# supranational/sppark

Hardware: AMD Instinct MI355X
Metric: MSM points/sec (BLS12-381 G1, 2^26 points) (higher is better)
Workload: dtype u32

## Files before the change

### sppark_amd/csrc/msm/msm_driver.hpp

```cpp
#pragma once
#include "msm_kernels.hpp"
#include "msm_coop_kernels.hpp"
#include "msm_route.hpp"
#include "../ec/jacobian_host.hpp"
#include "../util/runtime.hpp"
#include <algorithm>
#include <cmath>
#include <map>
#include <mutex>
#include <vector>

namespace sppark_amd {

template<class FD, class FH, class FRp>
class msm_t {
public:
    typedef FD fp_d;
    static constexpr bool G2_COOP_BUILT = field_is_internal<FD>::value && !field_is_montx<FD>::value;
    typedef mont_dev<FRp> fr_d;
    typedef FH fp_h;
    typedef typename xyzz_dev<fp_d>::mem_t bucket_t;
    typedef jacobian_host<fp_h> point_t;
    static constexpr int STD_WORDS = sizeof(FH) / 4;
    static constexpr size_t FP_BYTES = sizeof(FH);
    static constexpr bool INTERNAL = field_is_internal<FD>::value;
    static constexpr bool MONTX = field_is_montx<FD>::value;
    typedef xyzz_mem<STD_WORDS> std_bucket_t;
    static_assert(INTERNAL || sizeof(FH) == 4 * FD::N, "host and device coordinate fields must share the wire image");
    static constexpr size_t SCALAR_BYTES = sizeof(fr_d);
    static constexpr unsigned MAX_WINS = 128;
    static msm_field field()
    {
        bool pairs_default = false;
        if constexpr (G2_COOP_BUILT) pairs_default = fp_d::NL >= 14;
        return msm_field{INTERNAL, MONTX, G2_COOP_BUILT, pairs_default, (unsigned)fp_d::N, (unsigned)sizeof(bucket_t), (unsigned)FP_BYTES,
                         FRp::MOD, (unsigned)FRp::N};
    }
    static constexpr size_t FIXED_BASE_MIN = (size_t)1 << 23;

private:
    const gpu_info* gpu;
    hipStream_t stream;
    bool own_stream;
    hipStream_t aux = nullptr;
    unsigned gseq = 0;
    hipStream_t cpy = nullptr;
    hipEvent_t join_ev = nullptr;
    hipEvent_t ev_fork = nullptr, ev_sorted[2] = {nullptr, nullptr}, ev_accdone[2] = {nullptr, nullptr};
    hipEvent_t ev_copied[2] = {nullptr, nullptr}, ev_chunkdone[2] = {nullptr, nullptr};
    unsigned char* blob = nullptr;
    size_t blob_sz = 0;
    unsigned char* stage = nullptr;
    size_t stage_sz = 0;
    std_bucket_t* h_sums = nullptr;
    size_t h_sums_cap = 0;
    u32* h_flag = nullptr;
    const u32* h_flag_cur = nullptr;
    u32* d_pflag = nullptr;
    bool piece_pending = false;
    std::vector<hipEvent_t> tev;
    unsigned char* pre_points = nullptr;
    size_t pre_n = 0, pre_stride = 0;
    unsigned pre_fb_wbits = 0, pre_fb_nwins = 0;
    float last_ms[4] = {0, 0, 0, 0};
    unsigned last_chunks = 0;
    unsigned last_redo = 0;
    bool timing = false;

    struct layout {
        size_t digits[2], sorted[2], partA[2], H[2], tot[2], offA[2], off[2], curB[2], bigl[2];
        size_t buckets, keyA, ptA, keyB, ptB, keyC, flag, A1, W1, A2, W2, conv, sums, total;
    };

    static size_t align_up(size_t x) { return (x + 255) & ~(size_t)255; }
    static constexpr size_t conv_stride()
    {
        if constexpr (INTERNAL) return affine_loader<FD>::STRIDE; else return 0;
    }

    layout make_layout(const msm_plan& p, bool convert) const
    {
        layout l; size_t o = 0;
        auto take = [&](size_t sz) { size_t r = o; o += align_up(sz); return r; };
        const size_t wg = p.wpg;
        for (unsigned b = 0; b < 2; b++) {
            if (b == 1 && p.G == 1) {
                l.digits[1] = l.digits[0]; l.sorted[1] = l.sorted[0]; l.partA[1] = l.partA[0]; l.H[1] = l.H[0]; l.tot[1] = l.tot[0];
                l.offA[1] = l.offA[0]; l.off[1] = l.off[0]; l.curB[1] = l.curB[0]; l.bigl[1] = l.bigl[0];
                break;
            }
            l.digits[b] = take(wg * p.n * 4);
            l.sorted[b] = take(wg * p.n * 4);
            l.partA[b]  = take(wg * p.n * (p.IB ? 4 : 8));
            l.H[b]      = take(wg * p.nslabs * p.NA * 4);
            l.tot[b]    = take(wg * p.NA * 4);
            l.offA[b]   = take(wg * (p.NA + 1) * 4);
            l.off[b]    = take(wg * ((size_t)p.NB + 1) * 4);
            l.curB[b]   = take(wg * ((size_t)p.NB + 1) * 4);
            l.bigl[b]   = take((wg * p.NA + 1) * 4);
        }
        l.buckets = take((size_t)p.nwins * p.NB * sizeof(bucket_t));
        size_t nrecA = (size_t)2 * p.nwins * p.chunks_per_win;
        size_t nrecB = 2 * ((nrecA + p.F - 1) / p.F);
        l.keyA = take(nrecA * 4); l.ptA = take(nrecA * sizeof(bucket_t));
        l.keyB = take(nrecB * 4); l.ptB = take(nrecB * sizeof(bucket_t));
        l.keyC = take(nrecA * 4); l.flag = take(4);
        size_t n1 = (size_t)p.nwins * std::max<size_t>(p.NB / p.K1, lg2_floor(p.NB) + 1);
        l.A1 = take(n1 * sizeof(bucket_t)); l.W1 = take(n1 * sizeof(bucket_t));
        l.A2 = take(n1 * sizeof(bucket_t)); l.W2 = take(n1 * sizeof(bucket_t));
        l.conv = take(INTERNAL && convert ? (size_t)p.n * conv_stride() : 0);
        l.sums = take(((size_t)p.nwins + 1) * std::max(sizeof(std_bucket_t), sizeof(bucket_t)));
        l.total = o;
        return l;
    }

    void reserve(size_t sz)
    {
        if (sz <= blob_sz) return;
        if (blob) {
            HIP_OK(hipStreamSynchronize(stream));
            if (aux) HIP_OK(hipStreamSynchronize(aux));
            HIP_OK(hipFree(blob)); blob = nullptr; blob_sz = 0;
        }
        HIP_OK(dev_scratch_pool::malloc_or_drain((void**)&blob, sz));
        blob_sz = sz;
    }
    void reserve_stage(size_t sz)
    {
        if (sz <= stage_sz) return;
        if (stage) { HIP_OK(hipDeviceSynchronize()); HIP_OK(hipFree(stage)); stage = nullptr; stage_sz = 0; }
        HIP_OK(dev_scratch_pool::malloc_or_drain((void**)&stage, sz));
        stage_sz = sz;
    }
    void reserve_sums(size_t count)
    {
        if (count <= h_sums_cap) return;
        if (h_sums) { HIP_OK(hipStreamSynchronize(stream)); HIP_OK(hipHostFree(h_sums)); h_sums = nullptr; h_sums_cap = 0; }
        HIP_OK(hipHostMalloc((void**)&h_sums, count * sizeof(std_bucket_t), hipHostMallocDefault));
        h_sums_cap = count;
    }
    void need_event(hipEvent_t& e) { if (!e) HIP_OK(hipEventCreateWithFlags(&e, hipEventDisableTiming)); }
    std::map<const void*, size_t> lds_done;
    void lds_attr(const void* fn, size_t bytes)
    {
        size_t& have = lds_done[fn];
        if (bytes <= have) return;
        HIP_OK(hipFuncSetAttribute(fn, hipFuncAttributeMaxDynamicSharedMemorySize, (int)bytes));
        have = bytes;
    }
    void need_aux()
    {
        if (aux) return;
        unsigned ncu = 0;
#ifdef SPPARK_TUNING
        if (const char* e = getenv("SPPARK_MSM_AUX_CUS")) ncu = (unsigned)atoi(e);
#endif
        const unsigned total = (unsigned)gpu->prop.multiProcessorCount;
        hipError_t err = hipErrorNotSupported;
        if (ncu && ncu < total) {
            std::vector<uint32_t> mask((total + 31) / 32, 0);
            for (unsigned k = 0; k < ncu; k++) {
                unsigned cu = (unsigned)(((uint64_t)k * total) / ncu);
                mask[cu / 32] |= 1u << (cu % 32);
            }
            err = hipExtStreamCreateWithCUMask(&aux, (uint32_t)mask.size(), mask.data());
            if (err != hipSuccess) { (void)hipGetLastError(); aux = nullptr; }
        }
        if (!aux) HIP_OK(hipStreamCreateWithFlags(&aux, hipStreamNonBlocking));
        need_event(ev_fork);
        for (int b = 0; b < 2; b++) { need_event(ev_sorted[b]); need_event(ev_accdone[b]); }
    }
    void need_cpy()
    {
        if (cpy) return;
        HIP_OK(hipStreamCreateWithFlags(&cpy, hipStreamNonBlocking));
        for (int b = 0; b < 2; b++) { need_event(ev_copied[b]); need_event(ev_chunkdone[b]); }
    }
    void need_tev(size_t count)
    {
        while (tev.size() < count) { hipEvent_t e; HIP_OK(hipEventCreate(&e)); tev.push_back(e); }
    }

public:
    msm_tunables tune;

    explicit msm_t(int device_id = -1, hipStream_t s = nullptr)
        : gpu(&select_gpu(device_id)), stream(s), own_stream(false)
    {
        {
            int nb = 0, cur = -1;
            (void)hipGetDevice(&cur);
            if (cur != gpu->hip_id) HIP_OK(hipSetDevice(gpu->hip_id));
            if (hipOccupancyMaxActiveBlocksPerMultiprocessor(&nb, (const void*)k_accumulate<fp_d, false>, 256, 0) == hipSuccess && nb > 0)
                tune.resident_lanes = (size_t)std::min(nb, 2) * 256 * (size_t)gpu->prop.multiProcessorCount;
            else (void)hipGetLastError();
            if (cur >= 0 && cur != gpu->hip_id) (void)hipSetDevice(cur);
        }
        if constexpr (G2_COOP_BUILT) { if (fp_d::NL >= 14) tune.long_runs = 1; }
        if (stream == nullptr) {
            HIP_OK(hipStreamCreateWithFlags(&stream, hipStreamNonBlocking));
            HIP_OK(hipEventCreateWithFlags(&join_ev, hipEventDisableTiming));
            own_stream = true;
        }
    }
    ~msm_t()
    {
        int cur = -1;
        (void)hipGetDevice(&cur);
        if (cur != gpu->hip_id) (void)hipSetDevice(gpu->hip_id);
        (void)hipStreamSynchronize(stream);
        if (aux) (void)hipStreamSynchronize(aux);
        if (cpy) (void)hipStreamSynchronize(cpy);
        if (blob) (void)hipFree(blob);
        if (stage) (void)hipFree(stage);
        if (h_sums) (void)hipHostFree(h_sums);
        if (h_flag) (void)hipHostFree(h_flag);
        if (d_pflag) (void)hipFree(d_pflag);
        if (pre_points) (void)hipFree(pre_points);
        for (auto& e : tev) (void)hipEventDestroy(e);
        for (hipEvent_t e : {ev_fork, ev_sorted[0], ev_sorted[1], ev_accdone[0], ev_accdone[1],
                             ev_copied[0], ev_copied[1], ev_chunkdone[0], ev_chunkdone[1], join_ev})
            if (e) (void)hipEventDestroy(e);
        if (aux) (void)hipStreamDestroy(aux);
        if (cpy) (void)hipStreamDestroy(cpy);
        if (own_stream) (void)hipStreamDestroy(stream);
        if (cur >= 0 && cur != gpu->hip_id) (void)hipSetDevice(cur);
    }
    msm_t(const msm_t&) = delete;
    msm_t& operator=(const msm_t&) = delete;

    int device() const { return gpu->hip_id; }
    void set_stream(hipStream_t s)
    {
        (void)hipStreamSynchronize(stream);
        if (own_stream) { (void)hipStreamDestroy(stream); own_stream = false; }
        stream = s;
        if (stream == nullptr) {
            HIP_OK(hipStreamCreateWithFlags(&stream, hipStreamNonBlocking));
            if (!join_ev) HIP_OK(hipEventCreateWithFlags(&join_ev, hipEventDisableTiming));
            own_stream = true;
        }
    }
    void enable_timing(bool on) { timing = on; }
    float kernel_ms(int which) const { return which >= 0 && which < 4 ? last_ms[which] : -1.f; }
    unsigned chunks_of_last_invoke() const { return last_chunks; }
    unsigned tail_redone() const { return last_redo; }
    size_t scratch_bytes() const { return blob_sz + stage_sz; }
    void release_scratch()
    {
        (void)hipSetDevice(gpu->hip_id);
        (void)hipStreamSynchronize(stream);
        if (aux) (void)hipStreamSynchronize(aux);
        if (cpy) (void)hipStreamSynchronize(cpy);
        if (blob) { (void)hipFree(blob); blob = nullptr; blob_sz = 0; }
        if (stage) { (void)hipFree(stage); stage = nullptr; stage_sz = 0; }
    }
    msm_plan plan_for(size_t npoints) const { return make_plan(npoints, FRp::NBITS, tune); }

    void reserve_for(size_t npoints, size_t ffi_affine_sz, bool host_points, bool host_scalars)
    {
        HIP_OK(hipSetDevice(gpu->hip_id));
        size_t chunk = choose_chunk(npoints, (host_points ? ffi_affine_sz : 0) + (host_scalars ? SCALAR_BYTES : 0));
        const std::vector<size_t> cb = chunk_bounds(npoints, chunk);
        size_t need = 0;
        for (size_t c = 0; c + 1 < cb.size(); c++) need = std::max(need, make_layout(make_plan(cb[c + 1] - cb[c], FRp::NBITS, tune), true).total);
        reserve(need);
        if (host_points || host_scalars)
            reserve_stage(2 * (align_up(host_points ? chunk * ffi_affine_sz : 0) + align_up(host_scalars ? chunk * SCALAR_BYTES : 0)));
    }

    void join_default_stream()
    {
        if (!own_stream) return;
        HIP_OK(hipEventRecord(join_ev, nullptr));
        HIP_OK(hipStreamWaitEvent(stream, join_ev, 0));
    }

    unsigned fixed_base_width(size_t np) const
    {
        if (tune.wbits) return std::min(26u, std::max(8u, tune.wbits));
        unsigned w = 0; double best = 0;
        for (unsigned c = 8; c <= 26; c++) {
            const double cost = (double)((FRp::NBITS - 1) / c + 1) * (double)np + 3.0 * (double)((size_t)1 << (c - 1));
            if (w == 0 || cost < best) { best = cost; w = c; }
        }
        return w;
    }
    void preload(const void* points, size_t np, size_t ffi_affine_sz, bool fixed_base = false)
    {
        HIP_OK(hipSetDevice(gpu->hip_id));
        HIP_OK(hipStreamSynchronize(stream));
        join_default_stream();
        if (np != 0 && (points == nullptr || ffi_affine_sz < 2 * FP_BYTES || np > (1u << 31))) HIP_OK(hipErrorInvalidValue);
        if (np != 0 && fixed_base && !MONTX) HIP_OK(hipErrorNotSupported);
        if (np != 0 && fixed_base && (tune.wbits || np >= FIXED_BASE_MIN)
            && (size_t)((FRp::NBITS - 1) / fixed_base_width(np) + 1) * np >= ((size_t)1 << 31)) HIP_OK(hipErrorInvalidValue);
        if (pre_points) { HIP_OK(hipFree(pre_points)); pre_points = nullptr; pre_n = pre_stride = 0; }
        pre_fb_wbits = pre_fb_nwins = 0;
        if (np == 0) return;
        if (fixed_base && !MONTX) HIP_OK(hipErrorNotSupported);
        if (fixed_base && !tune.wbits && np < FIXED_BASE_MIN) fixed_base = false;
        unsigned fb_w = 0, fb_nw = 1;
        if (fixed_base) {
            fb_w = fixed_base_width(np);
            fb_nw = (FRp::NBITS - 1) / fb_w + 1;
            fb_w = FRp::NBITS / fb_nw + (FRp::NBITS % fb_nw ? 1 : 0);
            if ((size_t)fb_nw * np >= ((size_t)1 << 31)) HIP_OK(hipErrorInvalidValue);
        }
        if (points == nullptr || ffi_affine_sz < 2 * FP_BYTES || np > (1u << 31)) HIP_OK(hipErrorInvalidValue);
        struct dev_buf {
            unsigned char* p = nullptr;
            ~dev_buf() { if (p) (void)hipFree(p); }
        } staging;
        try {
            if constexpr (INTERNAL) {
                const unsigned char* src = (const unsigned char*)points;
                if (!is_device_pointer(points)) {
                    HIP_OK(hipMalloc((void**)&staging.p, np * ffi_affine_sz));
                    HIP_OK(hipMemcpyAsync(staging.p, points, np * ffi_affine_sz, hipMemcpyHostToDevice, stream));
                    src = staging.p;
                }
                HIP_OK(dev_scratch_pool::malloc_or_drain((void**)&pre_points, (size_t)fb_nw * np * conv_stride()));
                launch_convert(pre_points, src, (unsigned)np, ffi_affine_sz);
                if constexpr (MONTX) if (fixed_base) {
                    hipLaunchKernelGGL(k_fixed_base_table<fp_d>, dim3((unsigned)((np + 255) / 256)), dim3(256), 0, stream,
                                       pre_points, (unsigned)np, fb_nw, (unsigned)FRp::NBITS);
                    HIP_OK(hipGetLastError());
                }
            } else {
                HIP_OK(hipMalloc((void**)&pre_points, np * ffi_affine_sz));
                HIP_OK(hipMemcpyAsync(pre_points, points, np * ffi_affine_sz,
                                      is_device_pointer(points) ? hipMemcpyDeviceToDevice : hipMemcpyHostToDevice, stream));
            }
            HIP_OK(hipStreamSynchronize(stream));
        } catch (...) {
            if (pre_points) { (void)hipFree(pre_points); pre_points = nullptr; }
            throw;
        }
        pre_n = np; pre_stride = ffi_affine_sz;
        if (fixed_base) { pre_fb_wbits = fb_w; pre_fb_nwins = fb_nw; }
    }
    unsigned fixed_base_windows() const { return pre_fb_nwins; }
    size_t preloaded() const { return pre_n; }

private:
    static void no_kernel() { HIP_OK(hipErrorInvalidDeviceFunction); }
    void launch_convert(unsigned char* dst, const unsigned char* src, unsigned n, size_t stride, hipStream_t on = nullptr)
    {
        if constexpr (INTERNAL)
            issue_convert(route_convert(field(), tune.sw, n, stride, ((size_t)src & 15) == 0), dst, src, stride, on ? on : stream);
    }
    void issue_convert(const msm_step& s, unsigned char* dst, const unsigned char* src, size_t stride, hipStream_t on)
    {
        if constexpr (INTERNAL) {
            const dim3 grid(s.gx), block(s.block);
            switch (s.kernel) {
            case MK_CONVERT:         hipLaunchKernelGGL((k_convert_points<fp_d, false>), grid, block, 0, on, dst, src, s.count, (unsigned)stride); break;
            case MK_CONVERT_FLAGGED: hipLaunchKernelGGL((k_convert_points<fp_d, true>), grid, block, 0, on, dst, src, s.count, (unsigned)stride); break;
            case MK_CONVERT_STAGED:
                if constexpr (MONTX) hipLaunchKernelGGL((k_convert_points_staged<fp_d, false>), grid, block, 0, on, dst, src, s.count); else no_kernel();
                break;
            case MK_CONVERT_STAGED_FLAGGED:
                if constexpr (MONTX) hipLaunchKernelGGL((k_convert_points_staged<fp_d, true>), grid, block, 0, on, dst, src, s.count); else no_kernel();
                break;
            default: no_kernel();
            }
            HIP_OK(hipGetLastError());
        } else no_kernel();
    }

    size_t choose_chunk(size_t n, size_t stage_per_point) const
    {
        size_t chunk = n;
        if (tune.chunk) chunk = std::min(n, std::max<size_t>(tune.chunk, 1));
        else if (stage_per_point && n > ((size_t)1 << 21)) {
            chunk = std::min<size_t>(std::max<size_t>(n / 4, (size_t)1 << 20), (size_t)1 << 24);
        }
        auto need = [&](size_t c) {
            return make_layout(make_plan(c, FRp::NBITS, tune), true).total + 2 * c * stage_per_point + 1024;
        };
        size_t limit = tune.max_scratch;
        if (!limit) {
            const bool blob_ok = make_layout(make_plan(chunk, FRp::NBITS, tune), true).total <= blob_sz;
            const bool stage_ok = stage_per_point == 0 || 2 * (chunk * stage_per_point + 512) <= stage_sz;
            if (blob_ok && stage_ok) return chunk;
            size_t free_b = 0, total_b = 0;
            if (hipMemGetInfo(&free_b, &total_b) != hipSuccess) { (void)hipGetLastError(); return chunk; }
            limit = free_b - (free_b >> 5) + blob_sz + stage_sz;
        }
        while (need(chunk) > limit && chunk > 4096) chunk = (chunk + 1) / 2;
        return chunk;
    }

    std::vector<size_t> chunk_bounds(size_t n, size_t chunk) const
    {
        std::vector<size_t> b{0};
        for (size_t lo = chunk; lo < n; lo += chunk) b.push_back(lo);
        b.push_back(n);
        return b;
    }

    void sort_group(hipStream_t ss, const msm_plan& p, const layout& l, unsigned b, unsigned w0, unsigned wn,
                    const u32* d_scalars, bool mont, unsigned fb_n = 0, unsigned fb_nwins = 0)
    {
        u32* digits = (u32*)(blob + l.digits[b]);
        u32* sorted = (u32*)(blob + l.sorted[b]);
        u32* H = (u32*)(blob + l.H[b]);
        u32* tot = (u32*)(blob + l.tot[b]);
        u32* off = (u32*)(blob + l.off[b]);
        void* partA = blob + l.partA[b];
        u32* offA = (u32*)(blob + l.offA[b]);
        const bool packed = p.IB != 0;
        unsigned ngp = 1; while (ngp < p.NG) ngp <<= 1;
        const partA_fmt fmt{H, p.IB, p.SH, ngp, p.nslabs};
        const unsigned nlong = p.nbits % p.nwins, sf = nlong == 0 ? wn : (nlong > w0 ? std::min(wn, nlong - w0) : 0u);
        if (fb_n) {
            unsigned grid = std::min<unsigned>((fb_n + 255) / 256, 256 * 16);
            hipLaunchKernelGGL(k_breakdown<fr_d>, dim3(grid), dim3(256), 0, ss,
                               digits, d_scalars, fb_n, fb_nwins, (unsigned)FRp::NBITS, (int)mont, 0u, fb_nwins);
        } else {
            unsigned grid = std::min<unsigned>((p.n + 255) / 256, 256 * 16);
            hipLaunchKernelGGL(k_breakdown<fr_d>, dim3(grid), dim3(256), 0, ss,
                               digits, d_scalars, p.n, p.nwins, p.nbits, (int)mont, w0, wn);
        }
        HIP_OK(hipGetLastError());
        size_t ldsA = (size_t)p.NA * 4, ldsB = ((size_t)1 << p.LB) * 4 + SORT_NT * 4 + (size_t)SORTB_STAGE * 4 + PARTA_MAX_GROUPS * 4;
        if (ldsA > 65536) { lds_attr((const void*)k_histA, ldsA); lds_attr(packed ? (const void*)k_scatterA<true> : (const void*)k_scatterA<false>, ldsA); }
        if (ldsB > 65536) lds_attr(packed ? (const void*)k_sortB<true> : (const void*)k_sortB<false>, ldsB);
        hipLaunchKernelGGL(k_histA, dim3(p.nslabs, wn), dim3(SORT_NT), ldsA, ss,
                           H, digits, p.n, p.nslabs, p.slab_sz, p.NA, p.LB, sf);
        HIP_OK(hipGetLastError());
        size_t na_total = (size_t)wn * p.NA;
        hipLaunchKernelGGL(k_scan_slabs, dim3((unsigned)((na_total + 255) / 256)), dim3(256), 0, ss,
                           H, tot, p.nslabs, p.NA, wn);
        HIP_OK(hipGetLastError());
        hipLaunchKernelGGL(k_scan_parts, dim3(wn), dim3(1024), 0, ss, offA, tot, p.NA);
        HIP_OK(hipGetLastError());
        if (p.NA <= SCATA_MAX_NA && p.LB < 16) {
            const size_t ldsS = scatterA_staged_lds(p.NA);
            lds_attr(packed ? (const void*)k_scatterA_staged<true> : (const void*)k_scatterA_staged<false>, ldsS);
            if (packed) hipLaunchKernelGGL(k_scatterA_staged<true>, dim3(p.nslabs, wn), dim3(SORT_NT), ldsS, ss,
                                           (u32*)partA, digits, H, offA, p.n, p.nslabs, p.slab_sz, p.NA, p.LB, sf, p.IB);
            else        hipLaunchKernelGGL(k_scatterA_staged<false>, dim3(p.nslabs, wn), dim3(SORT_NT), ldsS, ss,
                                           (uint2*)partA, digits, H, offA, p.n, p.nslabs, p.slab_sz, p.NA, p.LB, sf, p.IB);
        } else {
            if (packed) hipLaunchKernelGGL(k_scatterA<true>, dim3(p.nslabs, wn), dim3(SORT_NT), ldsA, ss,
                                           (u32*)partA, digits, H, offA, p.n, p.nslabs, p.slab_sz, p.NA, p.LB, sf, p.IB);
            else        hipLaunchKernelGGL(k_scatterA<false>, dim3(p.nslabs, wn), dim3(SORT_NT), ldsA, ss,
                                           (uint2*)partA, digits, H, offA, p.n, p.nslabs, p.slab_sz, p.NA, p.LB, sf, p.IB);
        }
        HIP_OK(hipGetLastError());
        const unsigned big = tune.big ? tune.big : p.big ? p.big : (1u << 18);
        u32* nbig = (u32*)(blob + l.bigl[b]); u32* blist = nbig + 1; u32* curB = (u32*)(blob + l.curB[b]);
        const bool may_be_big = p.n > big;
        if (may_be_big) HIP_OK(hipMemsetAsync(nbig, 0, 4, ss));
        if (packed) hipLaunchKernelGGL(k_sortB<true>, dim3(p.NA, wn), dim3(SORT_NT), ldsB, ss,
                                       sorted, off, (const u32*)partA, offA, p.n, p.NA, p.LB, sf, big, fmt);
        else        hipLaunchKernelGGL(k_sortB<false>, dim3(p.NA, wn), dim3(SORT_NT), ldsB, ss,
                                       sorted, off, (const uint2*)partA, offA, p.n, p.NA, p.LB, sf, big, fmt);
        HIP_OK(hipGetLastError());
        if (!may_be_big) return;
        hipLaunchKernelGGL(k_big_find, dim3((p.NA * wn + 255) / 256), dim3(256), 0, ss,
                           nbig, blist, off, offA, p.NA, p.LB, sf, wn, big);
        size_t ldsBig = ((size_t)1 << p.LB) * 4;
        const size_t avg = (size_t)p.n / p.NA;
        const unsigned split = avg > big / 2 ? (unsigned)std::min<size_t>(SORTB_SPLIT, avg / (BIG_STAGE / 2) + 1) : SORTB_SPLIT;
        if (packed) hipLaunchKernelGGL(k_big_hist<true>, dim3(1024), dim3(1024), ldsBig, ss, off, (const u32*)partA, offA, nbig, blist, p.n, p.NA, p.LB, sf, split);
        else        hipLaunchKernelGGL(k_big_hist<false>, dim3(1024), dim3(1024), ldsBig, ss, off, (const uint2*)partA, offA, nbig, blist, p.n, p.NA, p.LB, sf, split);
        hipLaunchKernelGGL(k_big_scan, dim3(p.NA > 64 && avg > big / 2 ? 1024 : 64), dim3(1024), 0, ss, off, curB, offA, nbig, blist, p.NA, p.LB, sf);
        const size_t ldsSc = big_scatter_lds(p.LB);
        if (ldsSc > 65536) lds_attr(packed ? (const void*)k_big_scatter<true> : (const void*)k_big_scatter<false>, ldsSc);
        if (packed) hipLaunchKernelGGL(k_big_scatter<true>, dim3(1024), dim3(1024), ldsSc, ss, sorted, curB, (const u32*)partA, offA, nbig, blist, p.n, p.NA, p.LB, sf, split, fmt);
        else        hipLaunchKernelGGL(k_big_scatter<false>, dim3(1024), dim3(1024), ldsSc, ss, sorted, curB, (const uint2*)partA, offA, nbig, blist, p.n, p.NA, p.LB, sf, split, fmt);
        HIP_OK(hipGetLastError());
    }

    void enqueue(const msm_plan& p, const layout& l, const unsigned char* d_points, size_t stride, bool preconverted,
                 const u32* d_scalars, bool mont, std_bucket_t* h_out, bool first_timed, unsigned fb_n = 0, unsigned fb_nwins = 0,
                 bool redo = false, bool may_defer = false)
    {
        msm_call call;
        call.fb_n = fb_n; call.redo = redo; call.may_defer = may_defer;
        call.convert = INTERNAL && !preconverted;
        call.flagged = !preconverted && stride > 2 * FP_BYTES;
        call.stride = stride; call.aligned16 = ((size_t)d_points & 15) == 0;
#ifdef SPPARK_TUNING
        if (const char* e = getenv("SPPARK_TOP_CUT")) call.top_cut = (unsigned)atoi(e);
#endif
        const msm_route route = make_route(p, tune, field(), call);
        if (route.overflow) HIP_OK(hipErrorInvalidValue);
        const bool multi = p.G > 1;
        if (multi) need_aux();
        if (timing && first_timed && !redo) { need_tev(2 + 2 * p.G); HIP_OK(hipEventRecord(tev[0], stream)); }
        if (multi) {
            HIP_OK(hipEventRecord(ev_fork, stream));
            HIP_OK(hipStreamWaitEvent(aux, ev_fork, 0));
        }
        bucket_t* buckets = (bucket_t*)(blob + l.buckets);
        std_bucket_t* fin = (std_bucket_t*)(blob + l.sums);
        const u32* off0 = (const u32*)(blob + l.off[0]);
        auto rec = [&](msm_buf b) -> bucket_t* {
            switch (b) {
            case MB_BUCKETS: return buckets;
            case MB_PT_A: return (bucket_t*)(blob + l.ptA);
            case MB_PT_B: return (bucket_t*)(blob + l.ptB);
            case MB_A1: return (bucket_t*)(blob + l.A1);
            case MB_W1: return (bucket_t*)(blob + l.W1);
            case MB_A2: return (bucket_t*)(blob + l.A2);
            case MB_W2: return (bucket_t*)(blob + l.W2);
            default: return nullptr;
            }
        };
        auto key = [&](msm_buf b) -> u32* {
            return (u32*)(b == MB_KEY_A ? blob + l.keyA : b == MB_KEY_B ? blob + l.keyB : b == MB_KEY_C ? blob + l.keyC : nullptr);
        };
        auto flag_word = [&](msm_flag f) -> u32* { return f == MF_SCRATCH ? (u32*)(blob + l.flag) : f == MF_SMALL ? d_pflag : nullptr; };
        auto launch = [&](const msm_step& s, unsigned w0 = 0, unsigned wn = 0, unsigned b = 0) {
            const dim3 grid(s.gx, s.gy), block(s.block);
            bucket_t *r0 = rec(s.rd[0]), *r1 = rec(s.rd[1]), *w0p = rec(s.wr[0]), *w1p = rec(s.wr[1]);
            u32* flag = flag_word(s.flag);
            const u32* offp = multi ? (const u32*)nullptr : off0;
#define SPPARK_GO(kernel, ...) hipLaunchKernelGGL((kernel), grid, block, s.lds, stream, __VA_ARGS__)
#define SPPARK_GO_G1(kernel, ...) do { if constexpr (MONTX) SPPARK_GO(kernel, __VA_ARGS__); else no_kernel(); } while (0)
            switch (s.kernel) {
            case MK_CONVERT: case MK_CONVERT_FLAGGED: case MK_CONVERT_STAGED: case MK_CONVERT_STAGED_FLAGGED:
                issue_convert(s, blob + l.conv, d_points, stride, stream);
                return;
            case MK_ACCUMULATE: case MK_ACCUMULATE_FLAGGED: case MK_ACCUMULATE_G2C: {
                const u32* sorted = (const u32*)(blob + l.sorted[b]);
                const u32* off = (const u32*)(blob + l.off[b]);
                const dim3 rows(s.gx, wn);
                u32* keyA = key(MB_KEY_A); bucket_t* ptA = rec(MB_PT_A);
                if (s.kernel == MK_ACCUMULATE_G2C) {
                    if constexpr (G2_COOP_BUILT)
                        hipLaunchKernelGGL((k_accumulate_g2c<fp_d>), rows, block, 0, stream, buckets, keyA, ptA, d_points, (unsigned)stride,
                                           sorted, off, p.n, p.NB, p.L, p.chunks_per_win, w0);
                    else no_kernel();
                } else if (s.kernel == MK_ACCUMULATE_FLAGGED)
                    hipLaunchKernelGGL((k_accumulate<fp_d, true>), rows, block, 0, stream, buckets, keyA, ptA, d_points, (unsigned)stride,
                                       sorted, off, p.n, p.NB, p.L, p.chunks_per_win, w0);
                else
                    hipLaunchKernelGGL((k_accumulate<fp_d, false>), rows, block, 0, stream, buckets, keyA, ptA, d_points, (unsigned)stride,
                                       sorted, off, p.n, p.NB, p.L, p.chunks_per_win, w0);
                break;
            }
            case MK_PIECE_LEVEL:
                SPPARK_GO(k_piece_level<fp_d>, buckets, key(s.rd[0]), r1, off0, p.NB, p.L, p.chunks_per_win, p.nwins, route.piece_cmax, s.t, s.last, flag);
                break;
            case MK_PIECE_LEVEL_COOP:
                SPPARK_GO_G1(k_piece_level_coop<fp_d>, buckets, key(s.rd[0]), r1, off0, p.NB, p.L, p.chunks_per_win, p.nwins, route.piece_cmax, s.t, s.last, flag);
                break;
            case MK_PIECE_TAIL_COOP:
                SPPARK_GO_G1(k_piece_tail_coop<fp_d>, buckets, key(s.rd[0]), r1, off0, p.NB, p.L, p.chunks_per_win, p.nwins, route.piece_cmax, s.t, s.lgGB, flag);
                break;
            case MK_JOIN_RUNS:
                HIP_OK(hipMemsetAsync(flag, 0, 4, stream));
                SPPARK_GO(k_join_runs<fp_d>, buckets, key(s.wr[0]), key(s.rd[0]), r1, s.count, flag);
                break;
            case MK_REDUCE_RUNS:
                SPPARK_GO(k_reduce_runs<fp_d>, buckets, key(s.wr[0]), w1p, key(s.rd[0]), r1, s.count, s.fan, s.nthreads, (int)s.last, (const u32*)flag);
                break;
            case MK_REDUCE_RUNS_COOP:
                SPPARK_GO_G1(k_reduce_runs_coop<fp_d>, buckets, key(s.wr[0]), w1p, key(s.rd[0]), r1, s.count, s.fan, s.nthreads, 0, (const u32*)flag);
                break;
            case MK_REDUCE_TAIL:
                SPPARK_GO(k_reduce_tail<fp_d>, buckets, key(s.rd[0]), r1, key(s.wr[0]), w1p, s.count, s.fan, (const u32*)flag);
                break;
            case MK_REDUCE_TAIL_COOP:
                SPPARK_GO_G1(k_reduce_tail_coop<fp_d>, buckets, key(s.rd[0]), r1, key(s.wr[0]), w1p, s.count, s.fan, (const u32*)flag);
                break;
            case MK_BUCKET_SMALL_BITS_COOP: SPPARK_GO_G1(k_bucket_small_bits_coop<fp_d>, w0p, buckets, off0, p.NB, s.m); break;
            case MK_BUCKET_LEVEL1:      SPPARK_GO(k_bucket_level1<fp_d>, w0p, w1p, buckets, p.NB, s.fan, p.nwins, offp); break;
            case MK_BUCKET_LEVEL1_LAT:  SPPARK_GO_G1(k_bucket_level1_lat<fp_d>, w0p, w1p, buckets, p.NB, s.fan, p.nwins, offp); break;
            case MK_BUCKET_LEVEL1_PIPE: SPPARK_GO_G1(k_bucket_level1_pipe<fp_d>, w0p, w1p, buckets, p.NB, s.fan, p.nwins, offp); break;
            case MK_BUCKET_LEVEL1_COOP: SPPARK_GO_G1(k_bucket_level1_coop<fp_d>, w0p, w1p, buckets, p.NB, s.fan, p.nwins, offp); break;
            case MK_BUCKET_LEVELN:      SPPARK_GO(k_bucket_levelN<fp_d>, w0p, w1p, r0, r1, s.count, s.fan, s.lgG, p.nwins); break;
            case MK_BUCKET_LEVELN_LAT:  SPPARK_GO_G1(k_bucket_levelN_lat<fp_d>, w0p, w1p, r0, r1, s.count, s.fan, s.lgG, p.nwins); break;
            case MK_BUCKET_LEVELN_PIPE: SPPARK_GO_G1(k_bucket_levelN_pipe<fp_d>, w0p, w1p, r0, r1, s.count, s.fan, s.lgG, p.nwins); break;
            case MK_BUCKET_LEVELN_COOP: SPPARK_GO_G1(k_bucket_levelN_coop<fp_d>, w0p, w1p, r0, r1, s.count, s.fan, s.lgG, p.nwins); break;
            case MK_BUCKET_TOP_BITS:
                if (s.lds > 65536) lds_attr((const void*)k_bucket_top_bits<fp_d>, s.lds);
                SPPARK_GO(k_bucket_top_bits<fp_d>, w0p, r0, r1, s.count, s.m, s.lgG);
                break;
            case MK_BUCKET_TOP_SUM: SPPARK_GO(k_bucket_top_sum<fp_d>, w0p, r0, s.m); break;
            case MK_BUCKET_TOP_BITS_COOP:
                if constexpr (MONTX) { if (s.lds > 65536) lds_attr((const void*)k_bucket_top_bits_coop<fp_d>, s.lds); }
                SPPARK_GO_G1(k_bucket_top_bits_coop<fp_d>, w0p, r0, r1, s.count, s.m, s.lgG, s.sb, s.sp);
                break;
            case MK_BUCKET_TOP_SUM_COOP:
                SPPARK_GO_G1(k_bucket_top_sum_coop<fp_d>, w0p, r0, s.count, fin, flag, flag ? reinterpret_cast<u32*>(fin + p.nwins) : (u32*)nullptr);
                break;
            case MK_FINALIZE:
                if constexpr (INTERNAL) SPPARK_GO((k_finalize<fp_d, STD_WORDS>), fin, r0, p.nwins); else no_kernel();
                break;
            default: no_kernel();
            }
#undef SPPARK_GO_G1
#undef SPPARK_GO
            HIP_OK(hipGetLastError());
        };
        if (multi && !redo) HIP_OK(hipMemsetAsync(buckets, 0, (size_t)p.nwins * p.NB * sizeof(bucket_t), stream));

        for (unsigned g = 0; g < p.G && !redo; g++, gseq++) {
            const unsigned b = multi ? (gseq & 1) : 0, w0 = g * p.wpg, wn = std::min(p.wpg, p.nwins - w0);
            if (g == 0) {
                sort_group(stream, p, l, b, w0, wn, d_scalars, mont, fb_n, fb_nwins);
                if (call.convert) {
                    launch(route.steps[0]);
                    d_points = blob + l.conv;
                }
            } else {
                if (gseq >= 2) HIP_OK(hipStreamWaitEvent(aux, ev_accdone[b], 0));
                sort_group(aux, p, l, b, w0, wn, d_scalars, mont);
                HIP_OK(hipEventRecord(ev_sorted[b], aux));
                HIP_OK(hipStreamWaitEvent(stream, ev_sorted[b], 0));
            }
            if (timing && first_timed) HIP_OK(hipEventRecord(tev[2 + 2 * g], stream));
            launch(route.steps[route.front - 1], w0, wn, b);
            if (timing && first_timed) HIP_OK(hipEventRecord(tev[3 + 2 * g], stream));
            if (multi) HIP_OK(hipEventRecord(ev_accdone[b], stream));
        }

        unsigned si = route.front;
        piece_pending = route.piece_pending;
        if (route.flag_with_sums && !d_pflag) {
            HIP_OK(hipMalloc((void**)&d_pflag, 64));
            HIP_OK(hipMemsetAsync(d_pflag, 0, 64, stream));
        }
        if (route.pieces) {
            const msm_flag which = route.steps[si].flag;
            u32* flag = flag_word(which);
            if (which == MF_SCRATCH) HIP_OK(hipMemsetAsync(flag, 0, 4, stream));
            for (const unsigned end = si + route.pieces; si < end; si++) launch(route.steps[si]);
            if (!h_flag) HIP_OK(hipHostMalloc((void**)&h_flag, 64, hipHostMallocDefault));
            if (which == MF_SCRATCH) HIP_OK(hipMemcpyAsync(h_flag, flag, 4, hipMemcpyDeviceToHost, stream));
            h_flag_cur = which == MF_SMALL ? reinterpret_cast<const u32*>(h_out + p.nwins) : h_flag;
        }
        for (; si < route.nsteps && route.steps[si].kernel != MK_FINALIZE; si++) launch(route.steps[si]);
        if (timing && first_timed && !redo) HIP_OK(hipEventRecord(tev[1], stream));
        if constexpr (INTERNAL) {
            if (si < route.nsteps) launch(route.steps[si]);
            HIP_OK(hipMemcpyAsync(h_out, fin, (p.nwins + (route.flag_with_sums ? 1 : 0)) * sizeof(std_bucket_t), hipMemcpyDeviceToHost, stream));
        } else {
            HIP_OK(hipMemcpyAsync(h_out, rec(route.result), p.nwins * sizeof(std_bucket_t), hipMemcpyDeviceToHost, stream));
        }
    }

public:
    unsigned piece_tree_cmax(const msm_plan& p) const { return sppark_amd::piece_tree_cmax(p, tune.sw, 0, FRp::MOD, (unsigned)FRp::N); }
private:

    static point_t horner(const std_bucket_t* sums, const msm_plan& p)
    {
        point_t out; out.set_inf();
        for (unsigned w = p.nwins; w--;) {
            fp_h c[4];
            memcpy(c, &sums[w], sizeof(c));
            point_t s = point_t::from_xyzz(c[0], c[1], c[2], c[3]);
            out.add(s);
            if (w) for (unsigned k = 0; k < window_len(w - 1, p.nwins, p.nbits); k++) out.dbl();
        }
        return out;
    }

    msm_plan fixed_plan(size_t n) const
    {   return make_fixed_plan(n, pre_fb_wbits, pre_fb_nwins, SORTB_STAGE, tune);   }

    bool fixed_fits(size_t npoints, const void* scalars) const
    {
        const size_t need = make_layout(fixed_plan(npoints), false).total
                          + (is_device_pointer(scalars) ? 0 : 2 * align_up(npoints * SCALAR_BYTES));
        if (need <= blob_sz + stage_sz) return true;
        size_t free_b = 0, total_b = 0;
        if (hipMemGetInfo(&free_b, &total_b) != hipSuccess) { (void)hipGetLastError(); return true; }
        return need <= free_b - (free_b >> 5) + blob_sz + stage_sz;
    }

    void invoke_fixed(point_t& out, size_t npoints, const void* scalars, bool mont)
    {
        const msm_plan p = fixed_plan(npoints);
        const layout l = make_layout(p, false);
        const bool sc_dev = is_device_pointer(scalars);
        reserve(l.total);
        reserve_sums(MAX_WINS);
        const u32* d_scalars = (const u32*)scalars;
        if (!sc_dev) {
            reserve_stage(2 * align_up(npoints * SCALAR_BYTES));
            HIP_OK(hipMemcpyAsync(stage, scalars, npoints * SCALAR_BYTES, hipMemcpyHostToDevice, stream));
            d_scalars = (const u32*)stage;
        }
        enqueue(p, l, pre_points, conv_stride(), true, d_scalars, mont, h_sums, true, (unsigned)npoints, pre_fb_nwins);
        HIP_OK(hipStreamSynchronize(stream));
        last_chunks = 1;
        if (timing) {
            float acc = 0;
            HIP_OK(hipEventElapsedTime(&acc, tev[2], tev[3]));
            HIP_OK(hipEventElapsedTime(&last_ms[0], tev[0], tev[2]));
            last_ms[1] = acc;
            HIP_OK(hipEventElapsedTime(&last_ms[2], tev[0], tev[1]));
            last_ms[3] = 1.f;
        }
        out = horner(h_sums, p);
    }

public:
    void batch_add(point_t& out, const void* points, size_t npoints, const uint32_t* bitmap, const uint32_t* refmap,
                   size_t ffi_affine_sz)
    {
        out.set_inf();
        if (npoints == 0) return;
        if (npoints > (1u << 31) || !points || !bitmap || ffi_affine_sz < 2 * FP_BYTES) HIP_OK(hipErrorInvalidValue);
        HIP_OK(hipSetDevice(gpu->hip_id));
        join_default_stream();
        const size_t nwords = (npoints + 31) / 32;
        const unsigned span = 4;
        const size_t nrec = (nwords + span - 1) / span, F = 8;
        size_t o = 0;
        auto take = [&](size_t sz) { size_t r = o; o += align_up(sz); return r; };
        const bool pts_dev = is_device_pointer(points), bm_dev = is_device_pointer(bitmap), rm_dev = refmap && is_device_pointer(refmap);
        const size_t o_pts = take(pts_dev ? 0 : npoints * ffi_affine_sz), o_bm = take(bm_dev ? 0 : nwords * 4),
                     o_rm = take(refmap && !rm_dev ? nwords * 4 : 0), o_conv = take(INTERNAL ? npoints * conv_stride() : 0),
                     o_keyA = take(nrec * 4), o_ptA = take(nrec * sizeof(bucket_t)),
                     o_keyB = take((nrec / F + 2) * 2 * 4), o_ptB = take((nrec / F + 2) * 2 * sizeof(bucket_t)),
                     o_bucket = take(sizeof(bucket_t)), o_fin = take(sizeof(std_bucket_t));
        reserve(o);
        reserve_sums(1);
        const unsigned char* d_points = (const unsigned char*)points;
        const u32 *d_bm = bitmap, *d_rm = refmap;
        if (!pts_dev) { HIP_OK(hipMemcpyAsync(blob + o_pts, points, npoints * ffi_affine_sz, hipMemcpyHostToDevice, stream)); d_points = blob + o_pts; }
        if (!bm_dev) { HIP_OK(hipMemcpyAsync(blob + o_bm, bitmap, nwords * 4, hipMemcpyHostToDevice, stream)); d_bm = (const u32*)(blob + o_bm); }
        if (refmap && !rm_dev) { HIP_OK(hipMemcpyAsync(blob + o_rm, refmap, nwords * 4, hipMemcpyHostToDevice, stream)); d_rm = (const u32*)(blob + o_rm); }
        const bool flagged = ffi_affine_sz > 2 * FP_BYTES;
        if constexpr (INTERNAL) {
            launch_convert(blob + o_conv, d_points, (unsigned)npoints, ffi_affine_sz);
            d_points = blob + o_conv;
        }
        bucket_t* bucket = (bucket_t*)(blob + o_bucket);
        HIP_OK(hipMemsetAsync(bucket, 0, sizeof(bucket_t), stream));
        u32* ik = (u32*)(blob + o_keyA); bucket_t* ip = (bucket_t*)(blob + o_ptA);
        u32* ok = (u32*)(blob + o_keyB); bucket_t* op = (bucket_t*)(blob + o_ptB);
        {
            dim3 grid((unsigned)((nrec + 255) / 256));
            if (flagged) hipLaunchKernelGGL((k_bitmap_accumulate<fp_d, true>), grid, dim3(256), 0, stream, ik, ip, d_points,
                                            (unsigned)ffi_affine_sz, (unsigned)npoints, d_bm, d_rm, span);
            else         hipLaunchKernelGGL((k_bitmap_accumulate<fp_d, false>), grid, dim3(256), 0, stream, ik, ip, d_points,
                                            (unsigned)ffi_affine_sz, (unsigned)npoints, d_bm, d_rm, span);
            HIP_OK(hipGetLastError());
        }
        for (size_t n = nrec;;) {
            unsigned nthreads = (unsigned)((n + F - 1) / F);
            int last = nthreads == 1;
            hipLaunchKernelGGL(k_reduce_runs<fp_d>, dim3((nthreads + 255) / 256), dim3(256), 0, stream,
                               bucket, ok, op, ik, ip, (unsigned)n, (unsigned)F, nthreads, last, (const u32*)nullptr);
            HIP_OK(hipGetLastError());
            if (last) break;
            n = (size_t)2 * nthreads;
            std::swap(ik, ok); std::swap(ip, op);
        }
        if constexpr (INTERNAL) {
            std_bucket_t* fin = (std_bucket_t*)(blob + o_fin);
            hipLaunchKernelGGL((k_finalize<fp_d, STD_WORDS>), dim3(1), dim3(64), 0, stream, fin, bucket, 1u);
            HIP_OK(hipGetLastError());
            HIP_OK(hipMemcpyAsync(h_sums, fin, sizeof(std_bucket_t), hipMemcpyDeviceToHost, stream));
        } else {
            HIP_OK(hipMemcpyAsync(h_sums, bucket, sizeof(std_bucket_t), hipMemcpyDeviceToHost, stream));
        }
// ... 102 lines not shown
```

### sppark_amd/csrc/msm/msm_plan.hpp

```cpp
#pragma once
#include "msm_thresholds.hpp"
#include <algorithm>
#include <cstddef>

namespace sppark_amd {

struct msm_switches {
    bool no_join = false;
    bool no_narrow_end = false;
    bool no_latency_sums = false;
    bool no_coop = false;
    bool no_piece_tree = false;
    bool convert_per_lane = false;
    bool top_per_sum = false;
    bool piece_level_launches = false;
    bool sums_one_lane = false;
    size_t piece_fuse_max = PIECE_FUSE_MAX;
};

static inline bool decode_tail_code(unsigned code, msm_switches& s)
{
    s = msm_switches();
    if (code >= 16 + 64) return false;
    switch (code) {
    case 1:  s.no_join = s.no_piece_tree = true; break;
    case 2:  s.no_narrow_end = true; break;
    case 3:  s.no_latency_sums = true; break;
    case 4:  s.no_coop = true; break;
    case 5:  s.no_piece_tree = true; break;
    case 6:  s.convert_per_lane = true; break;
    case 7:  s.top_per_sum = true; break;
    case 8:  s.piece_level_launches = true; break;
    case 10: s.sums_one_lane = true; break;
    default: if (code >= 16) s.piece_fuse_max = (size_t)1 << (code - 16);
    }
    return true;
}

struct msm_plan {
    unsigned n, wbits, nwins, NB;
    unsigned nbits;
    unsigned HB, LB, NA;
    unsigned L, chunks_per_win;
    unsigned nslabs, slab_sz;
    unsigned F;
    unsigned K;
    unsigned K1;
    unsigned G, wpg;
    unsigned big;
    unsigned IB, SH, NG;
};

struct msm_tunables {
    unsigned wbits = 0, L = 0, F = 0, K = 0, nslabs = 0, LB = 0;
    unsigned big = 0;
    unsigned records = 0;
    unsigned groups = 0;
    unsigned top = 0;
    msm_switches sw;
    unsigned K1 = 0;
    unsigned g2_coop = 0;
    unsigned long_runs = 0;
    size_t resident_lanes = 0;
    size_t chunk = 0;
    size_t max_scratch = 0;
};

static inline unsigned lg2_floor(size_t x) { unsigned r = 0; while (x >>= 1) r++; return r; }

static inline msm_plan make_plan(size_t npoints, unsigned scalar_bits, const msm_tunables& t)
{
    msm_plan p;
    p.n = (unsigned)npoints;
    unsigned lg = lg2_floor(npoints ? npoints : 1);
    unsigned autow = lg >= 22 ? std::min(22u, lg - 4) : lg >= 19 ? 16u : lg == 18 ? 15u : lg == 17 ? 14u
                   : lg >= 14 ? 8u : std::max(4u, lg > 10 ? lg - 10 : 0u);
    p.wbits = t.wbits ? t.wbits : autow;
    p.wbits = std::min(24u, std::max(2u, p.wbits));
    p.nwins = (scalar_bits - 1) / p.wbits + 1;
    p.nbits = scalar_bits;
    p.wbits = scalar_bits / p.nwins + (scalar_bits % p.nwins ? 1 : 0);
    p.NB = 1u << (p.wbits - 1);
    const unsigned lgc = lg + ((npoints & (npoints - 1)) ? 1 : 0);
    unsigned hb = lgc > 14 ? lgc - 14 : 0;
    {
        const unsigned lgw = lg2_floor(p.nwins);
        hb = std::max(hb, lgw < 10 ? 10 - lgw : 0u);
        hb = std::min(hb, std::min(p.wbits - 1, 12u));
    }
    p.LB = t.LB ? std::min(t.LB, p.wbits - 1) : p.wbits - 1 - hb;
    if (p.LB > 13) p.LB = 13;
    if (p.wbits - 1 - p.LB > 15) p.LB = p.wbits - 1 - 15;
    p.HB = p.wbits - 1 - p.LB;
    p.NA = 1u << p.HB;
    size_t entries = (size_t)p.n * p.nwins;
    unsigned L = t.L ? t.L : lg >= 22 ? (lg >= 25 ? 256u : 128u)
                           : 1u << lg2_floor(std::min<size_t>(128, std::max<size_t>(8, entries / 131072)));
    const bool g2_runs = !t.L && t.long_runs && lg >= 16 && lg < 25;
    if (g2_runs) L = lg >= 20 ? 128u : lg >= 19 ? 64u : 32u;
    if (!t.L && !g2_runs && t.resident_lanes >= 256 && p.n >= 4096) {
        const size_t R = t.resident_lanes / 256, T0 = (size_t)p.nwins * (((p.n + L - 1) / L + 255) / 256);
        const size_t k_hi = (T0 + R - 1) / R, k_lo = k_hi > 1 ? k_hi - 1 : 1;
        if (k_hi >= 2 && k_hi <= 64) {
            size_t best_cost = 0; unsigned best_L = L;
            for (size_t k = k_lo; k <= k_hi; k++) {
                const size_t q = (k * R / p.nwins) * 256;
                if (q == 0) continue;
                const size_t Lk = (p.n + q - 1) / q;
                if (Lk < 4 || Lk > 1024) continue;
                const size_t cost = k * Lk * 100 + (k - k_lo) * 3 * Lk;
                if (best_cost == 0 || cost < best_cost) { best_cost = cost; best_L = (unsigned)Lk; }
            }
            if (best_cost && best_cost <= k_hi * (size_t)L * 92) L = best_L;
        }
    }
    p.L = L;
    p.chunks_per_win = (p.n + L - 1) / L;
    p.nslabs = t.nslabs ? t.nslabs
             : (unsigned)std::min<size_t>(64, std::max<size_t>(npoints / 131072, std::min<size_t>(8, std::max<size_t>(1, npoints / 2048))));
    p.slab_sz = (p.n + p.nslabs - 1) / p.nslabs;
    p.IB = p.SH = 0; p.NG = 1;
    if (t.records != 1 && (!t.nslabs || t.records == 2) && p.LB < 16) {
        const unsigned IB = 31 - p.LB;
        const unsigned lgs = std::min(lg2_floor(p.slab_sz ? p.slab_sz : 1), IB);
        const size_t ss = (size_t)1 << lgs, ns = (npoints + ss - 1) / ss, ng = (((ns ? ns : 1) - 1) >> (IB - lgs)) + 1;
        if (ng <= 128 && ns <= 129) { p.slab_sz = (unsigned)ss; p.nslabs = (unsigned)std::max<size_t>(1, ns); p.IB = IB; p.SH = IB - lgs; p.NG = (unsigned)ng; }
    }
    const bool joined = !t.sw.no_join && (size_t)p.n / p.NB <= (size_t)4 * p.L;
    p.F = std::max(4u, t.F ? t.F : (joined ? 16u : 4u));
    p.K = t.K ? t.K : (lg <= 22 ? 4 : 8);
    p.K = std::min(p.K, p.NB);
    p.K1 = std::min(t.K1 ? t.K1 : (p.NB >= (1u << 21) ? 16u : (p.NB == (1u << 15) || p.NB == (1u << 14)) ? 8u : p.NB == 128u ? 1u : p.K), p.NB);
    unsigned G = t.groups ? t.groups : 1u;
    G = std::max(1u, std::min(G, p.nwins));
    p.wpg = (p.nwins + G - 1) / G;
    p.G = (p.nwins + p.wpg - 1) / p.wpg;
    p.big = 0;
    return p;
}

static inline msm_plan make_fixed_plan(size_t n, unsigned fb_wbits, unsigned fb_nwins, unsigned register_stage, const msm_tunables& tune)
{
    msm_plan p;
    const size_t entries = (size_t)fb_nwins * n;
    const unsigned lg = lg2_floor(entries ? entries : 1);
    p.n = (unsigned)entries; p.wbits = fb_wbits; p.nwins = 1; p.nbits = fb_wbits;
    p.NB = 1u << (p.wbits - 1);
    unsigned hb = lg > 14 ? lg - 14 : 0;
    hb = std::min(std::max(hb, 10u), std::min(p.wbits - 1, 12u));
    p.LB = tune.LB ? std::min(tune.LB, p.wbits - 1) : p.wbits - 1 - hb;
    if (p.LB > 13) p.LB = 13;
    if (p.wbits - 1 - p.LB > 15) p.LB = p.wbits - 1 - 15;
    p.HB = p.wbits - 1 - p.LB; p.NA = 1u << p.HB;
    p.L = tune.L ? tune.L : 1u << lg2_floor(std::min<size_t>(256, std::max<size_t>(8, entries / 131072)));
    p.chunks_per_win = (p.n + p.L - 1) / p.L;
    p.nslabs = tune.nslabs ? tune.nslabs : (unsigned)std::min<size_t>(1024, std::max<size_t>(entries / 131072, std::min<size_t>(8, std::max<size_t>(1, entries / 2048))));
    p.slab_sz = (p.n + p.nslabs - 1) / p.nslabs;
    p.F = std::max(4u, tune.F ? tune.F : 8u);
    p.K = std::min(tune.K ? tune.K : 8u, p.NB);
    p.K1 = std::min(tune.K1 ? tune.K1 : (p.NB >= (1u << 21) ? 16u : p.NB == (1u << 15) ? 8u : p.K), p.NB);
    p.G = 1; p.wpg = 1;
    p.big = register_stage;
    p.IB = p.SH = 0; p.NG = 1;
    return p;
}

}
```

Baseline: 496.4 million.

## Hoist scalar breakdown out of window groups and share digits/offsets across groups

Scalar digit breakdown now runs once for all windows before the group loop, writing a full nwins*n digits array, instead of once per window group inside sort_group. Bucket offsets are likewise stored per window for all windows, so level-1 bucket kernels get real offsets even in the multi-group case, and the per-group bucket memset is dropped. This removes repeated scalar reads and breakdown launches when groups > 1, at the cost of a larger scratch allocation for digits and offsets. With the default single-group plan it mostly just moves the breakdown launch.

```diff
diff --git a/sppark_amd/csrc/msm/msm_driver.hpp b/sppark_amd/csrc/msm/msm_driver.hpp
--- a/sppark_amd/csrc/msm/msm_driver.hpp
+++ b/sppark_amd/csrc/msm/msm_driver.hpp
@@ -67,10 +67,7 @@
     unsigned last_redo = 0;
     bool timing = false;
 
-    struct layout {
-        size_t digits[2], sorted[2], partA[2], H[2], tot[2], offA[2], off[2], curB[2], bigl[2];
-        size_t buckets, keyA, ptA, keyB, ptB, keyC, flag, A1, W1, A2, W2, conv, sums, total;
-    };
+    typedef msm_layout layout;
 
     static size_t align_up(size_t x) { return (x + 255) & ~(size_t)255; }
     static constexpr size_t conv_stride()
@@ -80,38 +77,8 @@
 
     layout make_layout(const msm_plan& p, bool convert) const
     {
-        layout l; size_t o = 0;
-        auto take = [&](size_t sz) { size_t r = o; o += align_up(sz); return r; };
-        const size_t wg = p.wpg;
-        for (unsigned b = 0; b < 2; b++) {
-            if (b == 1 && p.G == 1) {
-                l.digits[1] = l.digits[0]; l.sorted[1] = l.sorted[0]; l.partA[1] = l.partA[0]; l.H[1] = l.H[0]; l.tot[1] = l.tot[0];
-                l.offA[1] = l.offA[0]; l.off[1] = l.off[0]; l.curB[1] = l.curB[0]; l.bigl[1] = l.bigl[0];
-                break;
-            }
-            l.digits[b] = take(wg * p.n * 4);
-            l.sorted[b] = take(wg * p.n * 4);
-            l.partA[b]  = take(wg * p.n * (p.IB ? 4 : 8));
-            l.H[b]      = take(wg * p.nslabs * p.NA * 4);
-            l.tot[b]    = take(wg * p.NA * 4);
-            l.offA[b]   = take(wg * (p.NA + 1) * 4);
-            l.off[b]    = take(wg * ((size_t)p.NB + 1) * 4);
-            l.curB[b]   = take(wg * ((size_t)p.NB + 1) * 4);
-            l.bigl[b]   = take((wg * p.NA + 1) * 4);
-        }
-        l.buckets = take((size_t)p.nwins * p.NB * sizeof(bucket_t));
-        size_t nrecA = (size_t)2 * p.nwins * p.chunks_per_win;
-        size_t nrecB = 2 * ((nrecA + p.F - 1) / p.F);
-        l.keyA = take(nrecA * 4); l.ptA = take(nrecA * sizeof(bucket_t));
-        l.keyB = take(nrecB * 4); l.ptB = take(nrecB * sizeof(bucket_t));
-        l.keyC = take(nrecA * 4); l.flag = take(4);
-        size_t n1 = (size_t)p.nwins * std::max<size_t>(p.NB / p.K1, lg2_floor(p.NB) + 1);
-        l.A1 = take(n1 * sizeof(bucket_t)); l.W1 = take(n1 * sizeof(bucket_t));
-        l.A2 = take(n1 * sizeof(bucket_t)); l.W2 = take(n1 * sizeof(bucket_t));
-        l.conv = take(INTERNAL && convert ? (size_t)p.n * conv_stride() : 0);
-        l.sums = take(((size_t)p.nwins + 1) * std::max(sizeof(std_bucket_t), sizeof(bucket_t)));
-        l.total = o;
-        return l;
+        return sppark_amd::make_layout(p, sizeof(bucket_t), std::max(sizeof(std_bucket_t), sizeof(bucket_t)),
+                                       INTERNAL && convert ? conv_stride() : 0);
     }
 
     void reserve(size_t sz)
@@ -400,20 +367,9 @@
         return b;
     }
 
-    void sort_group(hipStream_t ss, const msm_plan& p, const layout& l, unsigned b, unsigned w0, unsigned wn,
-                    const u32* d_scalars, bool mont, unsigned fb_n = 0, unsigned fb_nwins = 0)
-    {
-        u32* digits = (u32*)(blob + l.digits[b]);
-        u32* sorted = (u32*)(blob + l.sorted[b]);
-        u32* H = (u32*)(blob + l.H[b]);
-        u32* tot = (u32*)(blob + l.tot[b]);
-        u32* off = (u32*)(blob + l.off[b]);
-        void* partA = blob + l.partA[b];
-        u32* offA = (u32*)(blob + l.offA[b]);
-        const bool packed = p.IB != 0;
-        unsigned ngp = 1; while (ngp < p.NG) ngp <<= 1;
-        const partA_fmt fmt{H, p.IB, p.SH, ngp, p.nslabs};
-        const unsigned nlong = p.nbits % p.nwins, sf = nlong == 0 ? wn : (nlong > w0 ? std::min(wn, nlong - w0) : 0u);
+    void breakdown(hipStream_t ss, const msm_plan& p, const layout& l, const u32* d_scalars, bool mont, unsigned fb_n, unsigned fb_nwins)
+    {
+        u32* digits = (u32*)(blob + l.digits);
         if (fb_n) {
             unsigned grid = std::min<unsigned>((fb_n + 255) / 256, 256 * 16);
             hipLaunchKernelGGL(k_breakdown<fr_d>, dim3(grid), dim3(256), 0, ss,
@@ -421,9 +377,24 @@
         } else {
             unsigned grid = std::min<unsigned>((p.n + 255) / 256, 256 * 16);
             hipLaunchKernelGGL(k_breakdown<fr_d>, dim3(grid), dim3(256), 0, ss,
-                               digits, d_scalars, p.n, p.nwins, p.nbits, (int)mont, w0, wn);
+                               digits, d_scalars, p.n, p.nwins, p.nbits, (int)mont, 0u, p.nwins);
         }
         HIP_OK(hipGetLastError());
+    }
+
+    void sort_group(hipStream_t ss, const msm_plan& p, const layout& l, unsigned b, unsigned w0, unsigned wn)
+    {
+        const u32* digits = (const u32*)(blob + l.digits) + (size_t)w0 * p.n;
+        u32* sorted = (u32*)(blob + l.sorted[b]);
+        u32* H = (u32*)(blob + l.H[b]);
+        u32* tot = (u32*)(blob + l.tot[b]);
+        u32* off = (u32*)(blob + l.off) + (size_t)w0 * ((size_t)p.NB + 1);
+        void* partA = blob + l.partA[b];
+        u32* offA = (u32*)(blob + l.offA[b]);
+        const bool packed = p.IB != 0;
+        unsigned ngp = 1; while (ngp < p.NG) ngp <<= 1;
+        const partA_fmt fmt{H, p.IB, p.SH, ngp, p.nslabs};
+        const unsigned nlong = p.nbits % p.nwins, sf = nlong == 0 ? wn : (nlong > w0 ? std::min(wn, nlong - w0) : 0u);
         size_t ldsA = (size_t)p.NA * 4, ldsB = ((size_t)1 << p.LB) * 4 + SORT_NT * 4 + (size_t)SORTB_STAGE * 4 + PARTA_MAX_GROUPS * 4;
         if (ldsA > 65536) { lds_attr((const void*)k_histA, ldsA); lds_attr(packed ? (const void*)k_scatterA<true> : (const void*)k_scatterA<false>, ldsA); }
         if (ldsB > 65536) lds_attr(packed ? (const void*)k_sortB<true> : (const void*)k_sortB<false>, ldsB);
@@ -492,13 +463,14 @@
         const bool multi = p.G > 1;
         if (multi) need_aux();
         if (timing && first_timed && !redo) { need_tev(2 + 2 * p.G); HIP_OK(hipEventRecord(tev[0], stream)); }
+        if (!redo) breakdown(stream, p, l, d_scalars, mont, fb_n, fb_nwins);
         if (multi) {
             HIP_OK(hipEventRecord(ev_fork, stream));
             HIP_OK(hipStreamWaitEvent(aux, ev_fork, 0));
         }
         bucket_t* buckets = (bucket_t*)(blob + l.buckets);
         std_bucket_t* fin = (std_bucket_t*)(blob + l.sums);
-        const u32* off0 = (const u32*)(blob + l.off[0]);
+        const u32* off0 = (const u32*)(blob + l.off);
         auto rec = [&](msm_buf b) -> bucket_t* {
             switch (b) {
             case MB_BUCKETS: return buckets;
@@ -519,7 +491,6 @@
             const dim3 grid(s.gx, s.gy), block(s.block);
             bucket_t *r0 = rec(s.rd[0]), *r1 = rec(s.rd[1]), *w0p = rec(s.wr[0]), *w1p = rec(s.wr[1]);
             u32* flag = flag_word(s.flag);
-            const u32* offp = multi ? (const u32*)nullptr : off0;
 #define SPPARK_GO(kernel, ...) hipLaunchKernelGGL((kernel), grid, block, s.lds, stream, __VA_ARGS__)
 #define SPPARK_GO_G1(kernel, ...) do { if constexpr (MONTX) SPPARK_GO(kernel, __VA_ARGS__); else no_kernel(); } while (0)
             switch (s.kernel) {
@@ -528,7 +499,7 @@
                 return;
             case MK_ACCUMULATE: case MK_ACCUMULATE_FLAGGED: case MK_ACCUMULATE_G2C: {
                 const u32* sorted = (const u32*)(blob + l.sorted[b]);
-                const u32* off = (const u32*)(blob + l.off[b]);
+                const u32* off = off0 + (size_t)w0 * ((size_t)p.NB + 1);
                 const dim3 rows(s.gx, wn);
                 u32* keyA = key(MB_KEY_A); bucket_t* ptA = rec(MB_PT_A);
                 if (s.kernel == MK_ACCUMULATE_G2C) {
@@ -570,10 +541,10 @@
                 SPPARK_GO_G1(k_reduce_tail_coop<fp_d>, buckets, key(s.rd[0]), r1, key(s.wr[0]), w1p, s.count, s.fan, (const u32*)flag);
                 break;
             case MK_BUCKET_SMALL_BITS_COOP: SPPARK_GO_G1(k_bucket_small_bits_coop<fp_d>, w0p, buckets, off0, p.NB, s.m); break;
-            case MK_BUCKET_LEVEL1:      SPPARK_GO(k_bucket_level1<fp_d>, w0p, w1p, buckets, p.NB, s.fan, p.nwins, offp); break;
-            case MK_BUCKET_LEVEL1_LAT:  SPPARK_GO_G1(k_bucket_level1_lat<fp_d>, w0p, w1p, buckets, p.NB, s.fan, p.nwins, offp); break;
-            case MK_BUCKET_LEVEL1_PIPE: SPPARK_GO_G1(k_bucket_level1_pipe<fp_d>, w0p, w1p, buckets, p.NB, s.fan, p.nwins, offp); break;
-            case MK_BUCKET_LEVEL1_COOP: SPPARK_GO_G1(k_bucket_level1_coop<fp_d>, w0p, w1p, buckets, p.NB, s.fan, p.nwins, offp); break;
+            case MK_BUCKET_LEVEL1:      SPPARK_GO(k_bucket_level1<fp_d>, w0p, w1p, buckets, p.NB, s.fan, p.nwins, off0); break;
+            case MK_BUCKET_LEVEL1_LAT:  SPPARK_GO_G1(k_bucket_level1_lat<fp_d>, w0p, w1p, buckets, p.NB, s.fan, p.nwins, off0); break;
+            case MK_BUCKET_LEVEL1_PIPE: SPPARK_GO_G1(k_bucket_level1_pipe<fp_d>, w0p, w1p, buckets, p.NB, s.fan, p.nwins, off0); break;
+            case MK_BUCKET_LEVEL1_COOP: SPPARK_GO_G1(k_bucket_level1_coop<fp_d>, w0p, w1p, buckets, p.NB, s.fan, p.nwins, off0); break;
             case MK_BUCKET_LEVELN:      SPPARK_GO(k_bucket_levelN<fp_d>, w0p, w1p, r0, r1, s.count, s.fan, s.lgG, p.nwins); break;
             case MK_BUCKET_LEVELN_LAT:  SPPARK_GO_G1(k_bucket_levelN_lat<fp_d>, w0p, w1p, r0, r1, s.count, s.fan, s.lgG, p.nwins); break;
             case MK_BUCKET_LEVELN_PIPE: SPPARK_GO_G1(k_bucket_levelN_pipe<fp_d>, w0p, w1p, r0, r1, s.count, s.fan, s.lgG, p.nwins); break;
@@ -599,19 +570,18 @@
 #undef SPPARK_GO
             HIP_OK(hipGetLastError());
         };
-        if (multi && !redo) HIP_OK(hipMemsetAsync(buckets, 0, (size_t)p.nwins * p.NB * sizeof(bucket_t), stream));
 
         for (unsigned g = 0; g < p.G && !redo; g++, gseq++) {
             const unsigned b = multi ? (gseq & 1) : 0, w0 = g * p.wpg, wn = std::min(p.wpg, p.nwins - w0);
             if (g == 0) {
-                sort_group(stream, p, l, b, w0, wn, d_scalars, mont, fb_n, fb_nwins);
+                sort_group(stream, p, l, b, w0, wn);
                 if (call.convert) {
                     launch(route.steps[0]);
                     d_points = blob + l.conv;
                 }
             } else {
                 if (gseq >= 2) HIP_OK(hipStreamWaitEvent(aux, ev_accdone[b], 0));
-                sort_group(aux, p, l, b, w0, wn, d_scalars, mont);
+                sort_group(aux, p, l, b, w0, wn);
                 HIP_OK(hipEventRecord(ev_sorted[b], aux));
                 HIP_OK(hipStreamWaitEvent(stream, ev_sorted[b], 0));
             }
diff --git a/sppark_amd/csrc/msm/msm_plan.hpp b/sppark_amd/csrc/msm/msm_plan.hpp
--- a/sppark_amd/csrc/msm/msm_plan.hpp
+++ b/sppark_amd/csrc/msm/msm_plan.hpp
@@ -139,6 +139,48 @@
     return p;
 }
 
+struct msm_layout {
+    size_t digits, off;
+    size_t sorted[2], partA[2], H[2], tot[2], offA[2], curB[2], bigl[2];
+    size_t buckets, keyA, ptA, keyB, ptB, keyC, flag, A1, W1, A2, W2, conv, sums, total;
+};
+
+static inline msm_layout make_layout(const msm_plan& p, size_t bucket_bytes, size_t sum_bytes, size_t conv_stride)
+{
+    msm_layout l; size_t o = 0;
+    auto take = [&](size_t sz) { size_t r = o; o += (sz + 255) & ~(size_t)255; return r; };
+    const size_t wg = p.wpg;
+    l.digits = take((size_t)p.nwins * p.n * 4);
+    for (unsigned b = 0; b < 2; b++) {
+        if (b == 1 && p.G == 1) {
+            l.sorted[1] = l.sorted[0]; l.partA[1] = l.partA[0]; l.H[1] = l.H[0]; l.tot[1] = l.tot[0];
+            l.offA[1] = l.offA[0]; l.curB[1] = l.curB[0]; l.bigl[1] = l.bigl[0];
+            break;
+        }
+        l.sorted[b] = take(wg * p.n * 4);
+        l.partA[b]  = take(wg * p.n * (p.IB ? 4 : 8));
+        l.H[b]      = take(wg * p.nslabs * p.NA * 4);
+        l.tot[b]    = take(wg * p.NA * 4);
+        l.offA[b]   = take(wg * (p.NA + 1) * 4);
+        if (b == 0) l.off = take((size_t)p.nwins * ((size_t)p.NB + 1) * 4);
+        l.curB[b]   = take(wg * ((size_t)p.NB + 1) * 4);
+        l.bigl[b]   = take((wg * p.NA + 1) * 4);
+    }
+    l.buckets = take((size_t)p.nwins * p.NB * bucket_bytes);
+    const size_t nrecA = (size_t)2 * p.nwins * p.chunks_per_win;
+    const size_t nrecB = 2 * ((nrecA + p.F - 1) / p.F);
+    l.keyA = take(nrecA * 4); l.ptA = take(nrecA * bucket_bytes);
+    l.keyB = take(nrecB * 4); l.ptB = take(nrecB * bucket_bytes);
+    l.keyC = take(nrecA * 4); l.flag = take(4);
+    const size_t n1 = (size_t)p.nwins * std::max<size_t>(p.NB / p.K1, lg2_floor(p.NB) + 1);
+    l.A1 = take(n1 * bucket_bytes); l.W1 = take(n1 * bucket_bytes);
+    l.A2 = take(n1 * bucket_bytes); l.W2 = take(n1 * bucket_bytes);
+    l.conv = take((size_t)p.n * conv_stride);
+    l.sums = take(((size_t)p.nwins + 1) * sum_bytes);
+    l.total = o;
+    return l;
+}
+
 static inline msm_plan make_fixed_plan(size_t n, unsigned fb_wbits, unsigned fb_nwins, unsigned register_stage, const msm_tunables& tune)
 {
     msm_plan p;
```

After: 496.0 million, median of 2. No clear change (-0.1%).
